# SuperbTUM/Faster-Distributed-Training

Measured on AMD Instinct MI355X. Metric: images/sec (whole node) ResNet-50 bs=1024 DDP at 1/2/4/8 MI355X; epoch time, higher is better.
Workload: dtype bf16; 1 GPU; model=resnet50 (CIFAR stem, 10 classes), global_batch=1024, image_size=32, parallelism=dp1, optimizer=madgrad, mixup=input, native_kernels=True, hip_graphs=True, deterministic=False

## Files before the change

### csrc/api.h

```cpp
#pragma once
#include <cstdint>
#include <vector>

namespace fdt {
void act_affine_fwd(uint64_t x, uint64_t s, uint64_t t, uint64_t out, long M, int C, int act, float alpha, int dt_in,
                    int dt_out, uint64_t stream);
int stats_num_blocks(long M, int C);
void set_ew_unroll(bool on);
void channel_stats_partial(uint64_t y, uint64_t part, long M, int C, int dt, uint64_t stream);
void stats_finalize(uint64_t part, int nb, int C, double count, int mode, float eps, float momentum, uint64_t gamma,
                    uint64_t beta, uint64_t run_mean, uint64_t run_var, uint64_t nbt, uint64_t out_s, uint64_t out_t,
                    uint64_t save_mean, uint64_t save_aux, int zero_after, uint64_t stream);
void bn_frozen_coef(uint64_t table, int units, uint64_t out, uint64_t stream);
void act_bwd_reduce(uint64_t g, uint64_t x, uint64_t s, uint64_t t, uint64_t gx, uint64_t part, int part_rows, long M,
                    int C, int act, float alpha, int dt, uint64_t stream);
void reduce_partials(uint64_t part, int nb, int nq, int C, uint64_t out, int zero_after, uint64_t stream);
int partials_compact(uint64_t part, int nb, int W, int R, uint64_t out, uint64_t stream);
void stats_bwd_coef(uint64_t gs, uint64_t gt, int C, double count, int mode, float eps, uint64_t save_mean,
                    uint64_t save_aux, uint64_t gamma, uint64_t alpha, uint64_t beta, uint64_t ggamma, uint64_t gbeta,
                    uint64_t stream);
void stats_bwd_finalize(uint64_t part, int nb, int nq, int C, int a_mode, float a_eps, double a_count, uint64_t a_sm,
                        uint64_t a_sa, uint64_t a_gamma, uint64_t a_alpha, uint64_t a_beta, uint64_t a_gg,
                        uint64_t a_gb, int b_mode, float b_eps, double b_count, uint64_t b_sm, uint64_t b_sa,
                        uint64_t b_gamma, uint64_t b_alpha, uint64_t b_beta, uint64_t b_gg, uint64_t b_gb,
// ... 83 lines not shown
void colsum_bf16(uint64_t x, uint64_t out, long rows, int cols, long ld, uint64_t stream);
void slab_sum_acc(uint64_t src, uint64_t dst, int s, long ld, long n, uint64_t stream);
void relu_bwd_colsum(uint64_t gact, uint64_t pre, uint64_t gpre, uint64_t gb, long rows, int cols, int dt,
                     uint64_t stream);
void augment(uint64_t src, uint64_t idx, uint64_t labels_src, uint64_t labels_out, uint64_t out, int B, int H, int W,
             int C, int Cout, int pad, int do_flip, uint64_t rng, float m0, float m1, float m2, float s0, float s1,
             float s2, int nchw, int pad_norm, int dt_out, uint64_t stream);
void rng_advance(uint64_t rng, uint64_t stream);
void conv_igemm(uint64_t x, uint64_t x2, uint64_t ps, uint64_t pt, uint64_t pg, uint64_t w, uint64_t out, uint64_t part,
                int part_rows, uint64_t ex, uint64_t es, uint64_t et, uint64_t jmask, uint64_t jyb, uint64_t jout, long Nb, int Hi,
                int Wi, int Cx, int Ho, int Wo, int S, const std::vector<int>& dh, const std::vector<int>& dw,
                const std::vector<int>& wt, int Cout, int ldw, int Hout, int Wout, int OS, int oy, int ox, int pro,
                int pro_act, float pro_alpha, int epi, int epi_act, float epi_alpha, int BM, int BN, int BK, int nsplit,
                uint64_t slab, uint64_t cnt, int kg, uint64_t stream, const std::vector<uint64_t>& jz);
void conv_igemm_join(uint64_t y, uint64_t r, uint64_t s, uint64_t t, uint64_t s2, uint64_t t2, uint64_t w, uint64_t out,
                     uint64_t part, int part_rows, uint64_t jout, uint64_t jmask, long Nb, int H, int W, int Cx, int Cout,
                     int ldw, int BM, int BN, int BK, int nsplit, uint64_t slab, uint64_t cnt, int kg, uint64_t stream);
void ffn_gemm(uint64_t x, uint64_t w, uint64_t out, long M, int K, int N, int epi, uint64_t bias, uint64_t out2,
              uint64_t a_in, uint64_t gb, float p, uint64_t seed, uint64_t seed_ptr, int BM, int BN, int BK, int kg,
              uint64_t stream);
int conv_num_row_blocks(long M, int BM);
void set_conv_write_through(bool on);
void set_conv_debug_flags(int f);
std::vector<long> conv_splitk_workspace(long M, int Cout, int BM, int BN, int nsplit);
void conv_wgrad(uint64_t g, uint64_t y, uint64_t al, uint64_t be, uint64_t gs, uint64_t x, uint64_t xs, uint64_t xt,
                uint64_t slab,
                long Nb, int Hi, int Wi, int Cx, int Ho, int Wo, int S, const std::vector<int>& dh,
                const std::vector<int>& dw, int Cout, int ldw, int act, float act_alpha, int BM, int BN, int BK,
                int nsplit, int direct, int stages, uint64_t out, uint64_t cnt, int Cin, int accumulate,
                uint64_t stream);
void wgrad_reduce(uint64_t slab, uint64_t out, int nsplit, int Cout, int Cin, int ntaps, int Cxp, int accumulate,
                  uint64_t stream);
void conv_bwd_pair(uint64_t g, uint64_t y, uint64_t al, uint64_t be, uint64_t gs, uint64_t wd, uint64_t x, uint64_t xs,
                   uint64_t xt, uint64_t es, uint64_t et, uint64_t dx, uint64_t part, int part_rows, uint64_t dw,
                   uint64_t slab, long M, int Cin, int Cout, int epi, int act, int wgs, int accumulate,
                   uint64_t stream);
bool conv_bwd_pair_supported(int Cin, int Cout, int epi, int act, int xaff);
void pack_weights(const std::vector<uint64_t>& src, const std::vector<uint64_t>& wf, const std::vector<uint64_t>& wd,
                  const std::vector<int>& cout, const std::vector<int>& cin, const std::vector<int>& cxp,
                  const std::vector<int>& ntaps, uint64_t stream);
void jacobi_eigh(uint64_t A, uint64_t w, uint64_t V, uint64_t table, int batch, int n, int max_sweeps, float tol, uint64_t stream);
void attn_fwd(uint64_t q, uint64_t k, uint64_t v, const std::vector<long>& strides, uint64_t out, uint64_t out32,
              uint64_t lse, uint64_t mask, int B, int L, int H, float fill, float p_drop, uint64_t seed,
              uint64_t seed_ptr, uint64_t stream);
void attn_bwd(uint64_t q, uint64_t k, uint64_t v, const std::vector<long>& strides, uint64_t o32, uint64_t dout,
              uint64_t lse, uint64_t delta, uint64_t mask, uint64_t dq, uint64_t dk, uint64_t dv, int B, int L, int H,
// ... 32 lines not shown
```

### csrc/bindings.cpp

```cpp
#include <pybind11/pybind11.h>
#include <pybind11/stl.h>

#include "api.h"
#include "runtime/runtime_api.h"

namespace py = pybind11;

namespace fdt {
const char* source_hash();
}

PYBIND11_MODULE(_fdt_native, m) {
  m.doc() = "MI355X (gfx950) HIP kernels and native runtime of faster_distributed_training_amd";
  m.attr("arch") = "gfx950";
  m.def("source_hash", &fdt::source_hash, "sha256 of the csrc/ sources this binary was built from");
#define DEF(name) m.def(#name, &fdt::name)
  DEF(act_affine_fwd);
  DEF(stats_num_blocks);
  DEF(set_ew_unroll);
  DEF(channel_stats_partial);
  DEF(stats_finalize);
  DEF(bn_frozen_coef);
  DEF(act_bwd_reduce);
  DEF(reduce_partials);
  DEF(partials_compact);
  DEF(stats_bwd_coef);
  DEF(stats_bwd_finalize);
  DEF(affine_fold);
  DEF(residual_act_fwd);
  DEF(residual_act_bwd);
  DEF(set_deterministic_mode);
  DEF(deterministic_mode);
  DEF(conv_igemm);
  DEF(conv_igemm_join);
  DEF(ffn_gemm);
  DEF(conv_num_row_blocks);
  DEF(set_conv_write_through);
  DEF(set_conv_debug_flags);
  DEF(conv_splitk_workspace);
  DEF(conv_wgrad);
  DEF(wgrad_reduce);
  DEF(conv_bwd_pair);
  DEF(conv_bwd_pair_supported);
  DEF(pack_weights);
  DEF(jacobi_eigh);
  DEF(ngd_pre_eigh);
  DEF(ngd_sumsq);
  DEF(ngd_small_supported);
  DEF(ngd_small_proj);
  DEF(ngd_small_part_numel);
  DEF(ngd_proj_supported);
  DEF(ngd_mfma);
  DEF(ngd_proj);
  DEF(ngd_proj_hbuf_numel);
  DEF(ngd_rescale);
  DEF(ngd_gram_slab_numel);
  DEF(ngd_gram);
  DEF(ngd_wupdate);
  DEF(ngd_post_eigh);
  DEF(attn_fwd);
  DEF(attn_bwd);
// ... 50 lines not shown
```

### csrc/kernels/conv_h3.hip

```cpp
#include "conv_igemm_impl.h"

namespace fdt {
namespace conv {

constexpr int kH3Taps = 9;
constexpr int kH3Row = 16;

__device__ __forceinline__ void h3_dma16(__amdgpu_buffer_rsrc_t r, void* lds, uint32_t off) {
  __builtin_amdgcn_raw_ptr_buffer_load_lds(r, (__attribute__((address_space(3))) void*)lds, 16, off, 0, 0, 0);
}

template <int BM>
constexpr int h3_halo_rows_max() {
  return BM / 16 * 36;
}

struct H3Geom {
  int W, Rb, W2, bhr, NI, GW, SPR;
  __device__ __forceinline__ H3Geom(int W_, int H_, int BM) {
    W = W_;
    Rb = H_ < BM / W_ ? H_ : BM / W_;
    W2 = W_ + 2;
    GW = W_ < 16 ? W_ : 16;
    NI = 16 / GW;
    SPR = W_ / GW;
    int b = (Rb + 2) * W2;
    if (NI > 1) b += ((16 / NI) - b % 16 + 16) % 16;
    bhr = b;
  }
  __device__ __forceinline__ int pix(int blk, int n) const {
    const int pn = n < 4 ? n : n < 12 ? n + 12 : n < 16 ? n - 8 : n < 20 ? n + 8 : n < 28 ? n - 12 : n;
    const int s = blk * 2 + (pn >> 4), i = pn & 15;
    const int per = Rb * SPR;
    const int gi = s / per, rr = s - gi * per, r = rr / SPR, seg = rr - r * SPR;
    const int img = NI * gi + i / GW, col = seg * GW + i % GW;
    return img * (Rb * W) + r * W + col;
  }
  static __device__ __forceinline__ int elem(int q, int h) { return q * kH3Row + 8 * (h ^ ((q >> 3) & 1)); }
  __device__ __forceinline__ int halo_row(int p) const {
    const int b = p / (Rb * W), r = (p / W) % Rb, c = p % W;
    return b * bhr + (r + 1) * W2 + c + 1;
  }
};

template <int BM, int BN, int WM, int WN, int TP = kH3Taps>
constexpr size_t h3_stage_elems() { return (size_t)TP * BN * 16 + (size_t)h3_halo_rows_max<BM>() * kH3Row; }

template <int BM, int BN, int EPI, int ACT, int WM, int WN, bool DMA, int NS = 2, int TP = kH3Taps>
__global__ __launch_bounds__(64 * WM * WN, (NS == 1 || BN == 64) ? 4 : 1) void h3_kernel(const ConvArgs a) {
  static_assert(NS == 2 || (NS == 1 && DMA), "single-stage: LDS-DMA staging");
  constexpr int NT = 64 * WM * WN;
  constexpr int TN = BN / WN / 32, TM = BM / WM / 32;
  static_assert(TN >= 1 && TM >= 1, "wave tile >= 32x32");
  constexpr int WP = TP * BN * 2;
  constexpr int NWP = (WP + NT - 1) / NT;
  constexpr int HRM = h3_halo_rows_max<BM>();
  constexpr int NHP = (2 * HRM + NT - 1) / NT;
  constexpr int NQ = EPI == kEpiJoinBwd ? 3 : 2;
  constexpr int WTILE = TP * BN * 16;
  constexpr int STAGE = (int)h3_stage_elems<BM, BN, WM, WN, TP>();

  extern __shared__ __attribute__((aligned(16))) char smem[];
  float* red = reinterpret_cast<float*>(smem);
  int* ttab = reinterpret_cast<int*>(red + (NT / 64) * NQ * BN);
  constexpr int HDR = (((NT / 64) * NQ * BN + 2 * kH3Taps) * 4 + 15) & ~15;
  bf16* tiles = reinterpret_cast<bf16*>(smem + HDR);
// ... 317 lines not shown
```

### csrc/kernels/conv_igemm.hip

```cpp
#include "conv_igemm_impl.h"

#include <algorithm>

namespace fdt {

static void conv_igemm_impl(uint64_t x, uint64_t x2, uint64_t ps, uint64_t pt, uint64_t pg, uint64_t w, uint64_t out,
                            uint64_t part, int part_rows, uint64_t ex, uint64_t es, uint64_t et, uint64_t jmask,
                            uint64_t jyb, uint64_t jout, long Nb, int Hi, int Wi, int Cx, int Ho, int Wo, int S,
                            const std::vector<int>& dh, const std::vector<int>& dw, const std::vector<int>& wt, int Cout,
                            int ldw, int Hout, int Wout, int OS, int oy, int ox, int pro, int pro_act, float pro_alpha,
                            int epi, int epi_act, float epi_alpha, int BM, int BN, int BK, int nsplit, uint64_t slab,
                            uint64_t cnt, uint64_t pt2, uint64_t pout, uint64_t pmask, int kg, uint64_t stream,
                            const std::vector<uint64_t>& jz = {}) {
  using namespace conv;
  ConvArgs a{};
  a.pt2 = P<const float>(pt2);
  a.pout = P<bf16>(pout);
  a.pmask = P<uint8_t>(pmask);
  if (pro == kProJoin) {
    FDT_CHECK(x2 != 0 && pout != 0 && ps != 0 && pt != 0 && (pg == 0 || pt2 != 0),
              "join prologue: y, r, s, t, out");
    FDT_CHECK(dh.size() == 1 && S == 1 && Hi == Ho && Wi == Wo, "join prologue: 1x1 stride-1 convolution only");
  }
  a.x = P<const bf16>(x);
// ... 55 lines not shown
  {
    const int nkt = (a.K + BK - 1) / BK;
    if (nsplit < 1 || nkt <= 1) nsplit = 1;
    if (nsplit > nkt && nkt >= 1) nsplit = nkt;
    a.kps = nsplit == 1 ? (nkt > 1 ? nkt : 1) : (nkt + nsplit - 1) / nsplit;
    a.nsplit = nsplit == 1 ? 1 : (nkt + a.kps - 1) / a.kps;
    a.slab = P<float>(slab);
    a.cnt = P<int>(cnt);
    FDT_CHECK(a.nsplit == 1 || (slab != 0 && cnt != 0), "split-K needs a slab and a zeroed ticket buffer");
  }
  const bool pure = a.ntaps == 1 && dh[0] == 0 && dw[0] == 0 && wt[0] == 0 && S == 1 && Hi == Ho && Wi == Wo;
  hipStream_t st = as_stream(stream);
  if (a.M == 0) return;
  if (epi == kEpiNormAct) {
    FDT_CHECK(pro == kProNone && es != 0 && et != 0, "frozen epilogue: prologue-free, with scale and shift");
    FDT_CHECK(OS == 1 && oy == 0 && ox == 0 && Hout == Ho && Wout == Wo, "frozen epilogue: dense forward output");
  }
  const int act = (pro == kProAffineAct || pro == kProJoin)
                      ? pro_act
                      : ((epi == kEpiActBwd || epi == kEpiJoinBwd || epi == kEpiNormAct) ? epi_act : 0);
  if (kg >= 5 && kg <= 8) {
    FDT_CHECK(pro == kProNone && a.nsplit == 1, "kg 5-8 (halo 3x3): prologue-free, nsplit 1");
    FDT_CHECK(launch_h3(pro, epi, act, a, BM, BN, kg, st), "kg 5-8 (halo 3x3): unsupported tile / epilogue");
    return;
  }
  if (kg == 10) {
    FDT_CHECK(launch_x1(pro, epi, act, a, BM, BN, xn, pure, st),
              "kg 10 (stationary 1x1): 1x1 stride-1, prologue none / affine (ReLU, none) / fold, epilogue "
              "STATS / STORE / ADD / ReLU-mask JOINBWD, tile 128x128 | 64x128, K a multiple of 64 within LDS, "
              "xn dividing Cout / BN");
    return;
  }
  if (kg == 2 && a.nsplit > 1) kg = 1;
  if (kg == 3 && pro != kProNone) kg = 1;
  if (launch_cases_fwd(pro, epi, act, a, BM, BN, BK, kg, pure, st) ||
      launch_cases_fold(pro, epi, act, a, BM, BN, BK, kg, pure, st) ||
      launch_cases_join(pro, epi, act, a, BM, BN, BK, kg, pure, st) ||
      launch_cases_plain(pro, epi, act, a, BM, BN, BK, kg, pure, st) ||
      launch_cases_infer(pro, epi, act, a, BM, BN, BK, kg, pure, st) ||
      launch_cases_ffn(pro, epi, act, a, BM, BN, BK, kg, pure, st))
    return;
  FDT_CHECK(false, "unsupported (prologue, epilogue) combination");
}

void conv_igemm(uint64_t x, uint64_t x2, uint64_t ps, uint64_t pt, uint64_t pg, uint64_t w, uint64_t out, uint64_t part,
                int part_rows, uint64_t ex, uint64_t es, uint64_t et, uint64_t jmask, uint64_t jyb, uint64_t jout, long Nb, int Hi,
// ... 78 lines not shown
```

### csrc/kernels/conv_igemm_impl.h

```cpp
#pragma once
#include "common.h"
#include "bn_math.h"
#include "dropout_math.h"
#include <vector>

namespace fdt {
namespace conv {

typedef short bf16x8_t __attribute__((ext_vector_type(8)));
typedef float f32x16 __attribute__((ext_vector_type(16)));

enum Pro : int { kProNone = 0, kProAffineAct = 1, kProFold = 2, kProJoin = 3 };
enum Epi : int { kEpiStats = 0, kEpiActBwd = 1, kEpiStore = 2, kEpiAdd = 3, kEpiJoinBwd = 4, kEpiGeluFwd = 5,
                 kEpiGeluBwd = 6, kEpiNormAct = 7 };

struct ConvArgs {
  const bf16* x;
  const bf16* x2;
  const float* ps;
  const float* pt;
  const float* pg;
  const float* pt2;
  bf16* pout;
  uint8_t* pmask;
// ... 103 lines not shown
  return make_float4(__uint_as_float(v[0]), __uint_as_float(v[1]), __uint_as_float(v[2]), __uint_as_float(v[3]));
}

constexpr uint32_t kOOB = 0xFFFFFFF0u;

__device__ __forceinline__ void st_out(__amdgpu_buffer_rsrc_t r, uint32_t byte_off, bf16* p, const float* v, int wt) {
  if (wt) {
    u32x4_t u = {pack_bf16x2(v[0], v[1]), pack_bf16x2(v[2], v[3]), pack_bf16x2(v[4], v[5]), pack_bf16x2(v[6], v[7])};
    __builtin_amdgcn_raw_buffer_store_b128(u, r, byte_off, 0, 16);
  } else {
    Vec8<bf16>::store(p, v);
  }
}

template <int BM, int BN, int BK, int PRO, bool PURE>
constexpr int kMinWavesPerEU =
    (BM == 128 && BN == 128 && BK == 32 && (PRO == kProNone || (PRO == kProAffineAct && PURE))) ? 4
    : (BM == 128 && BN == 128 && (BK == 32 || (PRO != 2 && PRO != 3))) ? 3 : 1;

struct PixLinear {
  int wstride;
  __device__ __forceinline__ int operator()(int wm, int j, int n) const { return wm * wstride + j * 32 + n; }
};
template <int BM, int BN, int EPI, int ACT, int NT, int WM, int WN, class PixF = PixLinear>
__device__ __forceinline__ void conv_epilogue(const ConvArgs& a, f32x16 (&acc)[BN / WN / 32][BM / WM / 32], long m0,
                                              int n0, int bm, int tid, float* stg, float* red, bool ew,
                                              float inv_alpha, PixF pix = PixLinear{BM / WM}) {
  constexpr int TN = BN / WN / 32, TM = BM / WM / 32;
  constexpr int NQ = EPI == kEpiJoinBwd ? 3 : 2;
  constexpr int SW = BN + 4;
  constexpr int CG = BN / 8;
  constexpr int RPS = NT / CG;
  constexpr int NSW = WM * 32 / RPS;
  static_assert(NSW >= 1 && NSW * RPS == WM * 32, "epilogue sweep geometry");
  constexpr int NW = NT / 64;
  const int lane = tid & 63, wid = tid >> 6, wn = wid % WN, wm = wid / WN;
  constexpr bool STATS = EPI == kEpiStats || EPI == kEpiActBwd || EPI == kEpiJoinBwd;
  const int h = lane >> 5;
  const __amdgpu_buffer_rsrc_t ro = __builtin_amdgcn_make_buffer_rsrc(
      (void*)a.out, (short)0, (int)0xFFFFFFFF, 0x00020000);
  const int cg = tid % CG, rs = tid / CG;
  const int c = n0 + cg * 8;
  const bool dense = a.OS == 1 && a.oy == 0 && a.ox == 0 && a.Hout == a.Ho && a.Wout == a.Wo;
  float sv[8], tv[8];
  constexpr bool GELU = EPI == kEpiGeluFwd || EPI == kEpiGeluBwd;
  uint64_t dseed = 0;
  if constexpr (GELU) dseed = drop::live_seed(a.drop_seed, a.drop_seed_ptr);
  if constexpr (EPI == kEpiGeluFwd) {
    const float4* bp = reinterpret_cast<const float4*>(a.fbias + c);
    const float4 b0 = bp[0], b1 = bp[1];
// ... 42 lines not shown
    for (int sw = 0; sw < NSW; ++sw) {
      const int lr = rs + sw * RPS;
      const long m = m0 + pix(lr >> 5, j, lr & 31);
      if (ew && m < a.M) {
        uint32_t orow;
        if (dense) {
          orow = (uint32_t)m;
        } else {
          const int mi = (int)m, hw = a.Ho * a.Wo;
          const int n = mi / hw, rem = mi - n * hw;
          const int oh = rem / a.Wo, ow = rem - oh * a.Wo;
          orow = (uint32_t)((n * a.Hout + oh * a.OS + a.oy) * a.Wout + ow * a.OS + a.ox);
        }
        const uint32_t e = orow * (uint32_t)a.Cout + c;
        const float4 va = *reinterpret_cast<const float4*>(stg + lr * SW + cg * 8);
        const float4 vb = *reinterpret_cast<const float4*>(stg + lr * SW + cg * 8 + 4);
        float v[8] = {va.x, va.y, va.z, va.w, vb.x, vb.y, vb.z, vb.w};
        if constexpr (EPI == kEpiStats) {
#pragma unroll
          for (int k = 0; k < 8; ++k) { q0[k] += v[k]; q1[k] = fmaf(v[k], v[k], q1[k]); }
          st_out(ro, e * 2u, a.out + e, v, a.wthru);
        } else if constexpr (EPI == kEpiActBwd) {
          float x8[8];
          Vec8<bf16>::load(a.ex + e, x8);
#pragma unroll
          for (int k = 0; k < 8; ++k) {
            const float gp = v[k] * actg<ACT>(fmaf(x8[k], sv[k], tv[k]), inv_alpha);
            v[k] = gp * sv[k];
            q0[k] = fmaf(gp, x8[k], q0[k]);
            q1[k] += gp;
          }
          st_out(ro, e * 2u, a.out + e, v, a.wthru);
        } else if constexpr (EPI == kEpiJoinBwd) {
          float e8[8], ya[8], yb[8], o8[8];
          Vec8<bf16>::load(a.out + e, e8);
          Vec8<bf16>::load(a.ex + e, ya);
          const bool hb = a.jyb != nullptr;
          if (hb) Vec8<bf16>::load(a.jyb + e, yb);
          uint32_t mk = 0;
          if constexpr (ACT == kActRelu) mk = a.jmask[e >> 3];
          else if (!zm) Vec8<bf16>::load(a.jout + e, o8);
          else if (!hb) Vec8<bf16>::load(a.jx + e, o8);
#pragma unroll
          for (int k = 0; k < 8; ++k) {
            const float gv = v[k] + e8[k];
            float gp;
            if constexpr (ACT == kActRelu) {
// ... 637 lines not shown
  if constexpr (PRO == kProJoin) {
    FDT_T(64, 256, 64) FDT_T(128, 256, 32) FDT_T(128, 256, 64)
  }
#undef FDT_T
#undef FDT_T2
  FDT_CHECK(false, "unsupported conv tile");
}


bool launch_cases_fwd(int pro, int epi, int act, const ConvArgs& a, int BM, int BN, int BK, int kg, bool pure,
                      hipStream_t st);
bool launch_cases_fold(int pro, int epi, int act, const ConvArgs& a, int BM, int BN, int BK, int kg, bool pure,
                       hipStream_t st);
bool launch_cases_join(int pro, int epi, int act, const ConvArgs& a, int BM, int BN, int BK, int kg, bool pure,
                       hipStream_t st);
bool launch_cases_plain(int pro, int epi, int act, const ConvArgs& a, int BM, int BN, int BK, int kg, bool pure,
                        hipStream_t st);
bool launch_cases_ffn(int pro, int epi, int act, const ConvArgs& a, int BM, int BN, int BK, int kg, bool pure,
                      hipStream_t st);
bool launch_cases_infer(int pro, int epi, int act, const ConvArgs& a, int BM, int BN, int BK, int kg, bool pure,
                        hipStream_t st);
bool h3_supported(const ConvArgs& a, int BM);
bool launch_h3(int pro, int epi, int act, const ConvArgs& a, int BM, int BN, int kg, hipStream_t st);
bool x1_supported(int pro, int epi, int act, const ConvArgs& a, int BM, int BN, int xn, bool pure);
bool launch_x1(int pro, int epi, int act, const ConvArgs& a, int BM, int BN, int xn, bool pure, hipStream_t st);

}
}
```

### faster_distributed_training_amd/ops/conv_igemm.py

```python
from __future__ import annotations

import json
import os
from dataclasses import dataclass
from functools import lru_cache

import torch

from . import _native

PRO_NONE, PRO_AFFINE_ACT, PRO_FOLD, PRO_JOIN = 0, 1, 2, 3
EPI_STATS, EPI_ACTBWD, EPI_STORE, EPI_ADD, EPI_JOINBWD = 0, 1, 2, 3, 4
EPI_NORMACT = 7


def _sp():
    return _native.stream_ptr()


def _p(t):
    return 0 if t is None else t.data_ptr()


def pad_channels(c: int) -> int:
# ... 114 lines not shown
        return tile[0], tile[1], 64
    return tuple(tile[:3])


WG_STAGES = int(os.environ.get("FDT_WG_STAGES", "2"))
WG_FUSED_REDUCE = os.environ.get("FDT_WG_FUSED_REDUCE", "0") == "1"
WG_FUSED_MAX_SPLITS = 8

KGROUPS = os.environ.get("FDT_KGROUPS", "1") != "0"
KG_TILES = {(128, 128, 64), (128, 64, 64), (64, 128, 64), (64, 64, 64), (64, 64, 128)}


GLDS = os.environ.get("FDT_CONV_GLDS", "0") == "1"


LOOP = os.environ.get("FDT_CONV_LOOP", "old")

H3 = os.environ.get("FDT_CONV_H3", "1") == "1"
H3_MIN_TILES = int(os.environ.get("FDT_CONV_H3_MIN_TILES", "256"))
H3_TILES = {(256, 128), (256, 64), (128, 128)}
H3_LOOP = os.environ.get("FDT_CONV_H3_LOOP", "auto")
H3_KGS = (5, 6, 7, 8)
H3_S2 = os.environ.get("FDT_CONV_H3_S2", "0") == "1"


def _h3_kg(kg, W=8):
    if kg in H3_KGS:
        return kg
    return {"dma": 6, "dma64": 6, "auto": 6, "dma1": 7}.get(H3_LOOP, 5)


def h3_tile(N, H, W, shp: "ConvShape", pro, cout, force=False, cx=None, bn=None, s2cls=False):
    if cx is None:
        cx = shp.cxp
    conv_ok = shp.k == 3 and shp.pad == 1 and shp.stride == (2 if s2cls else 1)
    if not (H3 or force) or pro != PRO_NONE or cx % 16 or not conv_ok or W < 4 or W & (W - 1):
        return None
    bm = 256
    M = N * H * W
    if M % bm or bm % W:
        return None
    rb = min(H, bm // W)
    if (rb < H and H % rb) or (rb == H and bm % (H * W)):
        return None
    nbk, gw = bm // (rb * W), min(W, 16)
    ni = 16 // gw
    bhr = (rb + 2) * (W + 2)
    if ni > 1:
        bhr += ((16 // ni) - bhr % 16 + 16) % 16
        if nbk % ni or rb != H:
            return None
    elif W % 16:
        return None
    if nbk * bhr > bm // 16 * 36:
        return None
    if bn is None:
        bn = 64 if H3_LOOP == "dma64" else 128
    bn = bn if cout % bn == 0 else (64 if cout % 64 == 0 else 0)
    if not bn or (not force and (M // bm) * (cout // bn) < H3_MIN_TILES):
        return None
    return bm, bn


def h3_auto(N, H, W, shp: "ConvShape", pro, cout, cx=None):
    if H3_LOOP != "auto":
        t = h3_tile(N, H, W, shp, pro, cout, cx=cx)
        return None if t is None else (t, _h3_kg(None, W))
    if h3_tile(N, H, W, shp, pro, cout, force=True, cx=cx, bn=64) is None:
        return None
    tiles128 = (N * H * W // 256) * (cout // 128) if cout % 128 == 0 else 0
    if W >= 32:
        return (256, 64), 6
    if W >= 8:
        if tiles128 >= 512:
            return (256, 128), 7
        return ((256, 64), 6) if W >= 16 else None
    return ((256, 128), 6) if tiles128 >= 256 else None


def _loop_kg(ent, kgv):
    lp = (ent.get("loop") if ent else None) or LOOP
    return 4 if (kgv == 1 and lp == "rot") else kgv


X1_KG = 10
X1_BN = 128
X1_BM_OF_K = {64: 128, 128: 128, 256: 128, 512: 64}
X1_LDS_MAX = 80 * 1024


def x1_lds_bytes(pro, epi, K, bn=X1_BN):
    nprm = {PRO_FOLD: 3, PRO_AFFINE_ACT: 2}.get(pro, 0)
    nq = 3 if epi == EPI_JOINBWD else 2
    hdr = ((nprm * K + 4 * nq * bn) * 4 + 15) & ~15
# ... 83 lines not shown

def conv_fwd(x, wf, shp: ConvShape, s=None, t=None, act=0, alpha=1.0, tile=None, part=None, nsplit=None,
             fin=None, kg=None, norm=None, res=None, out_act=None, xn=None, out=None):
    nat = _native.native()
    N, H, W, C = x.shape
    assert C == shp.cxp and x.dtype == torch.bfloat16 and x.is_contiguous()
    Ho, Wo = out_hw(H, W, shp)
    M = N * Ho * Wo
    frozen = norm is not None
    if frozen:
        assert s is None and t is None and act == 0 and part is None and fin is None, \
            "frozen epilogue: prologue-free, no statistics"
        es, et = norm
        for v in (es, et):
            assert v.dtype == torch.float32 and v.is_contiguous() and v.numel() == shp.cout and v.device == x.device
        assert res is None or (res.dtype == torch.bfloat16 and res.is_contiguous() and res.device == x.device
                               and tuple(res.shape) == (N, Ho, Wo, shp.cout))
        oact, oalpha = out_act if out_act is not None else (0, 1.0)
    else:
        assert res is None and out_act is None, "res / out_act belong to the frozen epilogue (norm=)"
    pro = PRO_AFFINE_ACT if (s is not None or act != 0) else PRO_NONE
    ent = None
    h3 = None
    if kg in H3_KGS:
        t3 = h3_tile(N, H, W, shp, pro, shp.cout, True)
        h3 = None if t3 is None else (t3, kg)
    elif kg is None and tile is None and H3:
        h3 = h3_auto(N, H, W, shp, pro, shp.cout)
    if tile is None and h3 is None:
        ent = tuned(f"fwd{pro}", N, H, shp) or tuned("fwd", N, H, shp)
        tile = tuple(ent["tile"]) if ent else None
    if h3 is not None:
        ent, ((bm, bn), kgv), bk = {"loop": "old"}, h3, 16
        ns, slab_p, cnt_p = 1, 0, 0
    else:
        bm, bn, bk = _tile3(tile, M, shp.cout)
        if nsplit is not None:
            ent = dict(ent or {}, nsplit=nsplit) if frozen else {"nsplit": nsplit}
        ns, slab_p, cnt_p = _splitk_args(ent, M, shp.cout, shp.ntaps * C, bm, bn, bk, x.device)
        xn = int(xn if xn is not None else (ent or {}).get("xn", 1))
        x1 = x1_ok(_is_pure(shp), pro, EPI_NORMACT if frozen else EPI_STATS, int(act), shp.ntaps * C, shp.cout,
                   bm, bn, xn)
        kgv = _kg(ent, kg, (bm, bn, bk), ns, shp.ntaps * C, pro, x1)
    _log("fwd", N, H, shp, ent, (bm, bn, bk), ns, kgv)
    if kgv == X1_KG:
        ns, slab_p, cnt_p = xn, 0, 0
    if out is None:
        y = torch.empty(N, Ho, Wo, shp.cout, device=x.device, dtype=torch.bfloat16)
    else:
        y = out
        assert y.dtype == torch.bfloat16 and y.is_contiguous() and tuple(y.shape) == (N, Ho, Wo, shp.cout)
    dh, dw, wt = taps_fwd(shp.k, shp.pad)
    if frozen:
        nat.conv_igemm(x.data_ptr(), 0, 0, 0, 0, wf.data_ptr(), y.data_ptr(), 0, 0,
                       _p(res), es.data_ptr(), et.data_ptr(), 0, 0, 0,
                       N, H, W, C, Ho, Wo, shp.stride, list(dh), list(dw), list(wt), shp.cout, shp.ntaps * shp.cxp,
                       Ho, Wo, 1, 0, 0, PRO_NONE, 0, 1.0, EPI_NORMACT, int(oact), float(oalpha), bm, bn, bk, ns, slab_p,
                       cnt_p, _loop_kg(ent, kgv), _sp(), [])
        return y, None
    if part is None:
        part = stat_slots(2, shp.cout, x.device, M)
    if pro == PRO_AFFINE_ACT and s is None:
        s = torch.ones(C, device=x.device, dtype=torch.float32)
        t = torch.zeros(C, device=x.device, dtype=torch.float32)
    nat.conv_igemm(x.data_ptr(), 0, _p(s), _p(t), 0, wf.data_ptr(), y.data_ptr(), part.data_ptr(), part.shape[0],
                   0, 0, 0, 0, 0, 0,
                   N, H, W, C, Ho, Wo, shp.stride, list(dh), list(dw), list(wt), shp.cout, shp.ntaps * shp.cxp,
                   Ho, Wo, 1, 0, 0, pro, int(act), float(alpha), EPI_STATS, 0, 1.0, bm, bn, bk, ns, slab_p, cnt_p,
                   _loop_kg(ent, kgv), _sp(), [])
# ... 35 lines not shown

def conv_dgrad(g, y, al, be, wd, shp: ConvShape, x_shape, epi=EPI_STORE, out=None, ex=None, es=None, et=None,
               act=0, alpha=1.0, tile=None, part=None, nsplit=None, gs=None, jmask=None, jyb=None, jout=None,
               coef=None, kg=None, jz=None, xn=None):
    nat = _native.native()
    N, Hy, Wy, Cy = g.shape
    assert Cy == shp.cout and g.is_contiguous() and (y is None or y.is_contiguous())
    Nx, Hx, Wx, Cx = x_shape
    assert Cx == shp.cin
    if out is None:
        out = torch.empty(N, Hx, Wx, shp.cin, device=g.device, dtype=torch.bfloat16)
    if epi == EPI_ACTBWD and part is None:
        part = stat_slots(2, shp.cin, g.device, Nx * Hx * Wx)
    if epi == EPI_JOINBWD:
        assert shp.stride == 1 and ex is not None and part is not None and (
            jmask is not None or jout is not None or jz is not None)
        assert (jz is None) == (es is None), "z mode: es / et with jz"
        if jz is not None:
            assert act == 2 and et is not None and len(jz) == 3
            assert (jz[0] is not None and jz[1] is not None) if jyb is not None else jz[2] is not None
            if jz[2] is not None:
                assert jz[2].dtype == torch.bfloat16 and jz[2].is_contiguous() and tuple(jz[2].shape) == tuple(x_shape)
    ent = None
    h3ok = kg in H3_KGS or (kg is None and tile is None)
    if tile is None:
        pro = PRO_FOLD if al is not None else PRO_NONE
        e = EPI_STORE if epi in (EPI_ADD, EPI_JOINBWD) else epi
        ent = ((tuned(f"dgrad{pro}{epi}", N, Hx, shp) if e != epi else None)
               or tuned(f"dgrad{pro}{e}", N, Hx, shp) or tuned("dgrad", N, Hx, shp))
        tile = tuple(ent["tile"]) if ent else None
    if nsplit is not None:
        ent = {"nsplit": nsplit}
    classes = dgrad_classes(shp.k, shp.stride, shp.pad)
    assert coef is None or epi in (EPI_ACTBWD, EPI_JOINBWD)
    for (py, px, dh, dw, wt) in classes:
        Ha = (Hx - py + shp.stride - 1) // shp.stride
        Wa = (Wx - px + shp.stride - 1) // shp.stride
        M = N * Ha * Wa
        if len(dh) == 0 and epi == EPI_ADD:
            continue
        pro = PRO_FOLD if al is not None else PRO_NONE
        h3 = None
        if h3ok and epi in (EPI_ACTBWD, EPI_STORE) and len(dh) == 9:
            if kg in H3_KGS:
                t3 = h3_tile(N, Hx, Wx, shp, pro, shp.cin, True, cx=Cy)
                h3 = None if t3 is None else (t3, kg)
            elif H3:
                h3 = h3_auto(N, Hx, Wx, shp, pro, shp.cin, cx=Cy)
        elif (h3ok and epi in (EPI_ACTBWD, EPI_STORE) and len(dh) in (2, 4) and shp.k == 3 and shp.stride == 2
              and Ha == Hy and Wa == Wy and (H3_S2 or kg in H3_KGS)):
            t3 = h3_tile(N, Ha, Wa, shp, pro, shp.cin, force=kg in H3_KGS, cx=Cy, s2cls=True)
            h3 = None if t3 is None else (t3, 6)
        if h3 is not None:
            ((bm, bn), kgv), bk = h3, 16
            ns, slab_p, cnt_p = 1, 0, 0
        else:
            bm, bn, bk = _tile3(tile, M, shp.cin)
            ns, slab_p, cnt_p = _splitk_args(ent, M, shp.cin, len(dh) * Cy, bm, bn, bk, g.device)
            xnv = int(xn if xn is not None else (ent or {}).get("xn", 1))
            x1 = x1_ok(_is_pure(shp), pro, epi, int(act) if epi == EPI_JOINBWD else 0, len(dh) * Cy, shp.cin,
                       bm, bn, xnv, relu_mask=jmask is not None and jz is None)
            kgv = _kg(ent, kg, (bm, bn, bk), ns, len(dh) * Cy, pro, x1)
        _log("dgrad", N, Hx, shp, ent, (bm, bn, bk), ns, kgv)
        if kgv == X1_KG:
            ns, slab_p, cnt_p = xnv, 0, 0
        assert gs is None or pro == PRO_FOLD, "gs needs the fold prologue (al/be)"
        nat.conv_igemm(g.data_ptr(), _p(y) if pro == PRO_FOLD else 0, _p(al), _p(be), _p(gs), wd.data_ptr(),
                       out.data_ptr(), _p(part) if epi in (EPI_ACTBWD, EPI_JOINBWD) else 0,
                       part.shape[0] if part is not None else 0, _p(ex), _p(es), _p(et),
                       _p(jmask), _p(jyb), _p(jout), N, Hy, Wy, Cy, Ha, Wa, 1,
                       list(dh), list(dw), list(wt), shp.cin, shp.ntaps * shp.cout, Hx, Wx, shp.stride, py, px,
                       pro, 0, 1.0, epi, int(act), float(alpha), bm, bn, bk, ns, slab_p, cnt_p, _loop_kg(ent, kgv),
                       _sp(), [_p(v) for v in jz] if jz is not None else [])
    if coef is not None:
        _finalize_standalone(nat, 2, part, 3 if epi == EPI_JOINBWD else 2, shp.cin, coef[0], coef[1])
    return out, (part if epi in (EPI_ACTBWD, EPI_JOINBWD) else None)


WH3 = os.environ.get("FDT_WGRAD_H3", "1") == "1"
WH3_WGS = int(os.environ.get("FDT_WGRAD_H3_WGS", "256"))
WH3_MIN_CPS = int(os.environ.get("FDT_WGRAD_H3_MIN_CPS", "1"))
WH3_PX = 128
WH3_PIPE = os.environ.get("FDT_WGRAD_H3_PIPE", "0") == "1"
WH3_TS = int(os.environ.get("FDT_WGRAD_H3_TS", "1"))


def wh3_plan(N, H, W, shp: "ConvShape", cx, fold=False, xaff=False, force=False):
    if not (WH3 or force) or fold or xaff or shp.k != 3 or shp.stride != 1 or shp.pad != 1:
# ... 178 lines not shown
```

Before: 44150 images/sec.

## Add persistent halo 3x3 conv kernel with resident weights and double-buffered halo

Adds a persistent-grid 3x3 stride-1 conv kernel for 64->64 channel, 32-wide layers. Each CU-sized workgroup loads the full weight set into LDS once, then loops over tiles while DMA-prefetching the next tile's halo into a second buffer. For ACTBWD it also prefetches the epilogue activation input into registers. The kernel is selected automatically in h3_auto when there are enough tiles. This removes repeated weight loads and per-tile launch and prologue latency, at the cost of a large LDS footprint (one workgroup per CU) and fixed-shape restrictions.

```diff
diff --git a/csrc/api.h b/csrc/api.h
--- a/csrc/api.h
+++ b/csrc/api.h
@@ -129,6 +129,7 @@
 int conv_num_row_blocks(long M, int BM);
 void set_conv_write_through(bool on);
 void set_conv_debug_flags(int f);
+void set_conv_h3p_wgs(int wgs);
 std::vector<long> conv_splitk_workspace(long M, int Cout, int BM, int BN, int nsplit);
 void conv_wgrad(uint64_t g, uint64_t y, uint64_t al, uint64_t be, uint64_t gs, uint64_t x, uint64_t xs, uint64_t xt,
                 uint64_t slab,
diff --git a/csrc/bindings.cpp b/csrc/bindings.cpp
--- a/csrc/bindings.cpp
+++ b/csrc/bindings.cpp
@@ -37,6 +37,7 @@
   DEF(conv_num_row_blocks);
   DEF(set_conv_write_through);
   DEF(set_conv_debug_flags);
+  DEF(set_conv_h3p_wgs);
   DEF(conv_splitk_workspace);
   DEF(conv_wgrad);
   DEF(wgrad_reduce);
diff --git a/csrc/kernels/conv_h3.hip b/csrc/kernels/conv_h3.hip
--- a/csrc/kernels/conv_h3.hip
+++ b/csrc/kernels/conv_h3.hip
@@ -1,47 +1,12 @@
-#include "conv_igemm_impl.h"
+#include "conv_h3_geom.h"
 
 namespace fdt {
 namespace conv {
-
-constexpr int kH3Taps = 9;
-constexpr int kH3Row = 16;
-
-__device__ __forceinline__ void h3_dma16(__amdgpu_buffer_rsrc_t r, void* lds, uint32_t off) {
-  __builtin_amdgcn_raw_ptr_buffer_load_lds(r, (__attribute__((address_space(3))) void*)lds, 16, off, 0, 0, 0);
-}
 
 template <int BM>
 constexpr int h3_halo_rows_max() {
   return BM / 16 * 36;
 }
-
-struct H3Geom {
-  int W, Rb, W2, bhr, NI, GW, SPR;
-  __device__ __forceinline__ H3Geom(int W_, int H_, int BM) {
-    W = W_;
-    Rb = H_ < BM / W_ ? H_ : BM / W_;
-    W2 = W_ + 2;
-    GW = W_ < 16 ? W_ : 16;
-    NI = 16 / GW;
-    SPR = W_ / GW;
-    int b = (Rb + 2) * W2;
-    if (NI > 1) b += ((16 / NI) - b % 16 + 16) % 16;
-    bhr = b;
-  }
-  __device__ __forceinline__ int pix(int blk, int n) const {
-    const int pn = n < 4 ? n : n < 12 ? n + 12 : n < 16 ? n - 8 : n < 20 ? n + 8 : n < 28 ? n - 12 : n;
-    const int s = blk * 2 + (pn >> 4), i = pn & 15;
-    const int per = Rb * SPR;
-    const int gi = s / per, rr = s - gi * per, r = rr / SPR, seg = rr - r * SPR;
-    const int img = NI * gi + i / GW, col = seg * GW + i % GW;
-    return img * (Rb * W) + r * W + col;
-  }
-  static __device__ __forceinline__ int elem(int q, int h) { return q * kH3Row + 8 * (h ^ ((q >> 3) & 1)); }
-  __device__ __forceinline__ int halo_row(int p) const {
-    const int b = p / (Rb * W), r = (p / W) % Rb, c = p % W;
-    return b * bhr + (r + 1) * W2 + c + 1;
-  }
-};
 
 template <int BM, int BN, int WM, int WN, int TP = kH3Taps>
 constexpr size_t h3_stage_elems() { return (size_t)TP * BN * 16 + (size_t)h3_halo_rows_max<BM>() * kH3Row; }
diff --git a/csrc/kernels/conv_h3_geom.h b/csrc/kernels/conv_h3_geom.h
--- /dev/null
+++ b/csrc/kernels/conv_h3_geom.h
@@ -0,0 +1,43 @@
+#pragma once
+#include "conv_igemm_impl.h"
+
+namespace fdt {
+namespace conv {
+
+constexpr int kH3Taps = 9;
+constexpr int kH3Row = 16;
+
+__device__ __forceinline__ void h3_dma16(__amdgpu_buffer_rsrc_t r, void* lds, uint32_t off) {
+  __builtin_amdgcn_raw_ptr_buffer_load_lds(r, (__attribute__((address_space(3))) void*)lds, 16, off, 0, 0, 0);
+}
+
+struct H3Geom {
+  int W, Rb, W2, bhr, NI, GW, SPR;
+  __device__ __forceinline__ H3Geom(int W_, int H_, int BM) {
+    W = W_;
+    Rb = H_ < BM / W_ ? H_ : BM / W_;
+    W2 = W_ + 2;
+    GW = W_ < 16 ? W_ : 16;
+    NI = 16 / GW;
+    SPR = W_ / GW;
+    int b = (Rb + 2) * W2;
+    if (NI > 1) b += ((16 / NI) - b % 16 + 16) % 16;
+    bhr = b;
+  }
+  __device__ __forceinline__ int pix(int blk, int n) const {
+    const int pn = n < 4 ? n : n < 12 ? n + 12 : n < 16 ? n - 8 : n < 20 ? n + 8 : n < 28 ? n - 12 : n;
+    const int s = blk * 2 + (pn >> 4), i = pn & 15;
+    const int per = Rb * SPR;
+    const int gi = s / per, rr = s - gi * per, r = rr / SPR, seg = rr - r * SPR;
+    const int img = NI * gi + i / GW, col = seg * GW + i % GW;
+    return img * (Rb * W) + r * W + col;
+  }
+  static __device__ __forceinline__ int elem(int q, int h) { return q * kH3Row + 8 * (h ^ ((q >> 3) & 1)); }
+  __device__ __forceinline__ int halo_row(int p) const {
+    const int b = p / (Rb * W), r = (p / W) % Rb, c = p % W;
+    return b * bhr + (r + 1) * W2 + c + 1;
+  }
+};
+
+}
+}
diff --git a/csrc/kernels/conv_h3p.hip b/csrc/kernels/conv_h3p.hip
--- /dev/null
+++ b/csrc/kernels/conv_h3p.hip
@@ -0,0 +1,246 @@
+#include "conv_h3_geom.h"
+
+namespace fdt {
+namespace conv {
+
+namespace {
+constexpr int kPBM = 256, kPBN = 64, kPWM = 4, kPWN = 2, kPNT = 64 * kPWM * kPWN, kPTM = kPBM / kPWM / 32;
+constexpr int kPW = 32, kPRb = kPBM / kPW, kPW2 = kPW + 2, kPHR = (kPRb + 2) * kPW2;
+constexpr int kPC = 64, kPCh = kPC / 16;
+constexpr int kPHdr = 80;
+constexpr int kPWPlane = kH3Taps * kPBN * 16 * 2;
+constexpr int kPWBytes = kPCh * kPWPlane;
+constexpr int kPHPlane = kPHR * kH3Row * 2;
+constexpr int kPHPieces = kPCh * kPHR * 2;
+constexpr int kPHInstr = (kPHPieces + 63) / 64;
+constexpr int kPHBuf = kPHInstr * 1024;
+constexpr int kPStage = kPWM * 32 * (kPBN + 4) * 4;
+constexpr int kPRed = (kPNT / 64) * 2 * kPBN * 4;
+constexpr int kPLds = kPHdr + kPWBytes + 2 * kPHBuf;
+static_assert(kPStage + kPRed <= kPHBuf, "epilogue staging + statistics alias one halo buffer");
+static_assert(kPLds <= 160 * 1024, "LDS budget");
+static_assert(kPWPlane % 1024 == 0, "whole 1-KiB weight DMA pieces");
+
+struct PixH3P {
+  H3Geom g;
+  __device__ __forceinline__ int operator()(int wm_, int j, int n) const { return g.pix(wm_ + kPWM * j, n); }
+};
+
+int& h3p_wgs_ref() {
+  static int v = 0;
+  return v;
+}
+}
+
+template <int EPI, int ACT>
+__global__ __launch_bounds__(kPNT, 1) void h3p_kernel(const ConvArgs a) {
+  constexpr int NW = kPNT / 64;
+  const int ntiles = a.nbm;
+  if ((int)blockIdx.x >= ntiles) return;
+
+  extern __shared__ __attribute__((aligned(16))) char smem[];
+  int* ttab = reinterpret_cast<int*>(smem);
+  char* wts = smem + kPHdr;
+  char* ring = wts + kPWBytes;
+
+  const int tid = threadIdx.x, lane = tid & 63, wid = tid >> 6;
+  const int wn = wid % kPWN, wm = wid / kPWN;
+  const int wv = __builtin_amdgcn_readfirstlane(wid);
+  const float inv_alpha = ACT == kActCelu ? 1.f / a.epi_alpha : 1.f;
+  const H3Geom geo(kPW, a.Hi, kPBM);
+
+  if (tid < kH3Taps) {
+    ttab[tid] = a.wt[tid];
+    ttab[kH3Taps + tid] = a.dh[tid] * kPW2 + a.dw[tid];
+  }
+  __syncthreads();
+
+  const __amdgpu_buffer_rsrc_t rx_d = __builtin_amdgcn_make_buffer_rsrc((void*)a.x, (short)0,
+                                                                        (int)(a.Nb_HiWi_Cx_bytes), 0x00020000);
+  const __amdgpu_buffer_rsrc_t rw_d = __builtin_amdgcn_make_buffer_rsrc((void*)a.w, (short)0, (int)(a.w_bytes),
+                                                                        0x00020000);
+
+  {
+    constexpr int IPP = kPWPlane / 1024;
+#pragma unroll
+    for (int j = 0; j < kPCh * IPP / NW; ++j) {
+      const int wi = j * NW + wv;
+      const int ch = wi / IPP, piece = (wi - ch * IPP) * 64 + lane;
+      const int tap = piece / (2 * kPBN), rem = piece - tap * 2 * kPBN;
+      const int n = rem >> 1, lh = (rem & 1) ^ ((n >> 3) & 1);
+      const uint32_t src = ((uint32_t)n * (uint32_t)a.ldw + (uint32_t)(ttab[tap] * kPC + 16 * ch + 8 * lh)) * 2u;
+      h3_dma16(rw_d, wts + wi * 1024, src);
+    }
+  }
+  static_assert(kPCh * (kPWPlane / 1024) % NW == 0, "weight pieces divide over the waves");
+
+  constexpr int NHJ = (kPHInstr + NW - 1) / NW;
+  int hpk[NHJ];
+#pragma unroll
+  for (int j = 0; j < NHJ; ++j) {
+    const int piece = (j * NW + wv) * 64 + lane;
+    const int ch = piece / (2 * kPHR), rem = piece - ch * 2 * kPHR;
+    const int q = rem >> 1, part = (rem & 1) ^ ((q >> 3) & 1);
+    const int hr = q / kPW2, hc = q - hr * kPW2;
+    const bool v = piece < kPHPieces && hc >= 1 && hc <= kPW;
+    const int cls = !v ? 0 : hr == 0 ? 2 : hr == kPRb + 1 ? 3 : 1;
+    hpk[j] = (((hr - 1) * kPW + hc - 1) * (kPC * 2) + ch * 32 + part * 16) | cls;
+  }
+  const int hmask = (a.Hi >> 3) - 1;
+  auto issue = [&](int tile, int buf) {
+    const uint32_t base = (uint32_t)tile * (uint32_t)(kPBM * kPC * 2);
+    const int tr = tile & hmask;
+    const bool top = tr == 0, bot = tr == hmask;
+    char* dst = ring + buf * kPHBuf;
+#pragma unroll
+    for (int j = 0; j < NHJ; ++j) {
+      const int wi = j * NW + wv;
+      if (wi < kPHInstr) {
+        const int cls = hpk[j] & 3;
+        const bool ok = cls == 1 || (cls == 2 && !top) || (cls == 3 && !bot);
+        h3_dma16(rx_d, dst + wi * 1024, ok ? base + (uint32_t)(hpk[j] & ~15) : kOOB);
+      }
+    }
+  };
+
+  const int h = lane >> 5;
+  int xoff[kH3Taps][kPTM];
+#pragma unroll
+  for (int j = 0; j < kPTM; ++j) {
+    const int qb = geo.halo_row(geo.pix(wm + kPWM * j, lane & 31));
+#pragma unroll
+    for (int t = 0; t < kH3Taps; ++t) xoff[t][j] = H3Geom::elem(qb + ttab[kH3Taps + t], h) * 2;
+  }
+  const int arow = wn * 32 + (lane & 31);
+  const int aoff = (arow * 16 + 8 * (h ^ ((lane >> 3) & 1))) * 2;
+
+  constexpr bool PRE = EPI == kEpiActBwd;
+  constexpr int NEX = PRE ? 2 * kPTM : 1;
+  int exoff[NEX];
+  if constexpr (PRE) {
+    const PixH3P px{geo};
+#pragma unroll
+    for (int j = 0; j < kPTM; ++j)
+#pragma unroll
+      for (int sw = 0; sw < 2; ++sw) {
+        const int lr = tid / (kPBN / 8) + sw * (kPNT / (kPBN / 8));
+        exoff[j * 2 + sw] = px(lr >> 5, j, lr & 31) * kPBN + (tid % (kPBN / 8)) * 8;
+      }
+  }
+  static_assert(kPWM * 32 / (kPNT / (kPBN / 8)) == 2, "two sweeps per epilogue pass");
+
+  const bool no_dma = a.dbg & 2, no_mma = a.dbg & 4, no_epi = a.dbg & 8;
+  const int grid = gridDim.x;
+  issue(xcd_remap(blockIdx.x, ntiles), 0);
+  asm volatile("s_waitcnt vmcnt(0)" ::: "memory");
+  __syncthreads();
+  for (int k = 0;; ++k) {
+    const int vb = blockIdx.x + k * grid;
+    const int tile = xcd_remap(vb, ntiles);
+    const int buf = k & 1;
+    const bool more = vb + grid < ntiles;
+    if (more && !no_dma) issue(xcd_remap(vb + grid, ntiles), buf ^ 1);
+    ExRegs<NEX> exq;
+    if constexpr (PRE) {
+      const bf16* exb = a.ex + (long)tile * (kPBM * kPBN);
+#pragma unroll
+      for (int i = 0; i < NEX; ++i) exq.u[i] = *reinterpret_cast<const uint4*>(exb + exoff[i]);
+    }
+
+    f32x16 acc[1][kPTM];
+#pragma unroll
+    for (int j = 0; j < kPTM; ++j)
+#pragma unroll
+      for (int r = 0; r < 16; ++r) acc[0][j][r] = 0.f;
+
+    const char* Hl = ring + buf * kPHBuf;
+    bf16x8_t wf[2], xf[2][kPTM];
+    auto fetch = [&](int s, int sl) {
+      const int c = s / kH3Taps, t = s - c * kH3Taps;
+      wf[sl] = *reinterpret_cast<const bf16x8_t*>(wts + c * kPWPlane + t * (kPBN * 32) + aoff);
+#pragma unroll
+      for (int j = 0; j < kPTM; ++j)
+        xf[sl][j] = *reinterpret_cast<const bf16x8_t*>(Hl + c * kPHPlane + xoff[t][j]);
+    };
+    if (!no_mma) {
+    fetch(0, 0);
+#pragma unroll
+    for (int s = 0; s < kPCh * kH3Taps; ++s) {
+      const int sl = s & 1;
+      if (s + 1 < kPCh * kH3Taps) fetch(s + 1, sl ^ 1);
+      __builtin_amdgcn_sched_barrier(0);
+#pragma unroll
+      for (int j = 0; j < kPTM; ++j)
+        acc[0][j] = __builtin_amdgcn_mfma_f32_32x32x16_bf16(wf[sl], xf[sl][j], acc[0][j], 0, 0, 0);
+      __builtin_amdgcn_sched_barrier(0);
+    }
+    }
+
+    asm volatile("s_waitcnt vmcnt(0)" ::: "memory");
+    char* stg = ring + buf * kPHBuf;
+    if (no_epi) __syncthreads();
+    else if constexpr (PRE)
+      conv_epilogue<kPBM, kPBN, EPI, ACT, kPNT, kPWM, kPWN, PixH3P, ExRegs<NEX>>(
+          a, acc, (long)tile * kPBM, 0, tile, tid, reinterpret_cast<float*>(stg),
+          reinterpret_cast<float*>(stg + kPStage), true, inv_alpha, PixH3P{geo}, exq);
+    else
+      conv_epilogue<kPBM, kPBN, EPI, ACT, kPNT, kPWM, kPWN, PixH3P>(
+          a, acc, (long)tile * kPBM, 0, tile, tid, reinterpret_cast<float*>(stg),
+          reinterpret_cast<float*>(stg + kPStage), true, inv_alpha, PixH3P{geo});
+    if (!more) break;
+    asm volatile("s_waitcnt lgkmcnt(0)" ::: "memory");
+    __builtin_amdgcn_s_barrier();
+    asm volatile("" ::: "memory");
+  }
+}
+
+template <int EPI, int ACT>
+static void h3p_launch_one(const ConvArgs& a, int grid, hipStream_t st) {
+  auto kern = h3p_kernel<EPI, ACT>;
+  static bool attr = false;
+  if (!attr) {
+    FDT_HIP_CHECK(hipFuncSetAttribute(reinterpret_cast<const void*>(kern), hipFuncAttributeMaxDynamicSharedMemorySize,
+                                      kPLds));
+    attr = true;
+  }
+  hipLaunchKernelGGL(kern, dim3(grid), dim3(kPNT), kPLds, st, a);
+  FDT_LAUNCH_CHECK();
+}
+
+bool h3p_supported(int pro, int epi, int act, const ConvArgs& a, int BM, int BN) {
+  if (pro != kProNone || BM != kPBM || BN != kPBN || a.ntaps != kH3Taps || !h3_supported(a, BM)) return false;
+  if (a.Cx != kPC || a.Cout != kPBN || a.Wi != kPW || a.Hi < kPRb || (a.Hi & (a.Hi - 1)) != 0) return false;
+  return ((epi == kEpiStats || epi == kEpiStore) && act == kActNone) ||
+         (epi == kEpiActBwd && (act == kActRelu || act == kActCelu)) ||
+         (epi == kEpiNormAct && (act == kActNone || act == kActRelu || act == kActCelu));
+}
+
+bool launch_h3p(int pro, int epi, int act, const ConvArgs& a, int BM, int BN, hipStream_t st) {
+  if (!h3p_supported(pro, epi, act, a, BM, BN)) return false;
+  static int cus = 0;
+  if (cus == 0) {
+    int dev = 0;
+    FDT_HIP_CHECK(hipGetDevice(&dev));
+    FDT_HIP_CHECK(hipDeviceGetAttribute(&cus, hipDeviceAttributeMultiprocessorCount, dev));
+    FDT_CHECK(cus > 0, "persistent halo 3x3 conv: CU count");
+  }
+  const int want = h3p_wgs_ref() > 0 ? h3p_wgs_ref() : cus;
+  const int grid = want < a.nbm || h3p_wgs_ref() > 0 ? want : a.nbm;
+#define FDT_H3P(E_, A_) \
+  if (epi == E_ && act == A_) { h3p_launch_one<E_, A_>(a, grid, st); return true; }
+  FDT_H3P(kEpiStats, kActNone)
+  FDT_H3P(kEpiActBwd, kActRelu)
+  FDT_H3P(kEpiActBwd, kActCelu)
+  FDT_H3P(kEpiStore, kActNone)
+  FDT_H3P(kEpiNormAct, kActNone)
+  FDT_H3P(kEpiNormAct, kActRelu)
+  FDT_H3P(kEpiNormAct, kActCelu)
+#undef FDT_H3P
+  return false;
+}
+
+}
+
+void set_conv_h3p_wgs(int wgs) { conv::h3p_wgs_ref() = wgs > 0 ? wgs : 0; }
+
+}
diff --git a/csrc/kernels/conv_igemm.hip b/csrc/kernels/conv_igemm.hip
--- a/csrc/kernels/conv_igemm.hip
+++ b/csrc/kernels/conv_igemm.hip
@@ -101,6 +101,12 @@
   if (kg >= 5 && kg <= 8) {
     FDT_CHECK(pro == kProNone && a.nsplit == 1, "kg 5-8 (halo 3x3): prologue-free, nsplit 1");
     FDT_CHECK(launch_h3(pro, epi, act, a, BM, BN, kg, st), "kg 5-8 (halo 3x3): unsupported tile / epilogue");
+    return;
+  }
+  if (kg == 11) {
+    FDT_CHECK(a.nsplit == 1 && launch_h3p(pro, epi, act, a, BM, BN, st),
+              "kg 11 (persistent halo 3x3): dense 3x3 stride-1, 64 -> 64 channels, 32-wide images of a power-of-two "
+              "height >= 8, tile 256x64, prologue-free, epilogue STATS / STORE / ACTBWD / NORMACT");
     return;
   }
   if (kg == 10) {
diff --git a/csrc/kernels/conv_igemm_impl.h b/csrc/kernels/conv_igemm_impl.h
--- a/csrc/kernels/conv_igemm_impl.h
+++ b/csrc/kernels/conv_igemm_impl.h
@@ -149,10 +149,23 @@
   int wstride;
   __device__ __forceinline__ int operator()(int wm, int j, int n) const { return wm * wstride + j * 32 + n; }
 };
-template <int BM, int BN, int EPI, int ACT, int NT, int WM, int WN, class PixF = PixLinear>
+struct ExLoad {
+  static constexpr bool kPre = false;
+  __device__ __forceinline__ void get(int, float*) const {}
+};
+template <int NR>
+struct ExRegs {
+  static constexpr bool kPre = true;
+  uint4 u[NR];
+  __device__ __forceinline__ void get(int i, float* v) const {
+    v[0] = bf16_lo(u[i].x); v[1] = bf16_hi(u[i].x); v[2] = bf16_lo(u[i].y); v[3] = bf16_hi(u[i].y);
+    v[4] = bf16_lo(u[i].z); v[5] = bf16_hi(u[i].z); v[6] = bf16_lo(u[i].w); v[7] = bf16_hi(u[i].w);
+  }
+};
+template <int BM, int BN, int EPI, int ACT, int NT, int WM, int WN, class PixF = PixLinear, class ExQ = ExLoad>
 __device__ __forceinline__ void conv_epilogue(const ConvArgs& a, f32x16 (&acc)[BN / WN / 32][BM / WM / 32], long m0,
                                               int n0, int bm, int tid, float* stg, float* red, bool ew,
-                                              float inv_alpha, PixF pix = PixLinear{BM / WM}) {
+                                              float inv_alpha, PixF pix = PixLinear{BM / WM}, const ExQ& exq = ExQ{}) {
   constexpr int TN = BN / WN / 32, TM = BM / WM / 32;
   constexpr int NQ = EPI == kEpiJoinBwd ? 3 : 2;
   constexpr int SW = BN + 4;
@@ -241,7 +254,8 @@
           st_out(ro, e * 2u, a.out + e, v, a.wthru);
         } else if constexpr (EPI == kEpiActBwd) {
           float x8[8];
-          Vec8<bf16>::load(a.ex + e, x8);
+          if constexpr (ExQ::kPre) exq.get(j * NSW + sw, x8);
+          else Vec8<bf16>::load(a.ex + e, x8);
 #pragma unroll
           for (int k = 0; k < 8; ++k) {
             const float gp = v[k] * actg<ACT>(fmaf(x8[k], sv[k], tv[k]), inv_alpha);
@@ -925,6 +939,8 @@
                         hipStream_t st);
 bool h3_supported(const ConvArgs& a, int BM);
 bool launch_h3(int pro, int epi, int act, const ConvArgs& a, int BM, int BN, int kg, hipStream_t st);
+bool h3p_supported(int pro, int epi, int act, const ConvArgs& a, int BM, int BN);
+bool launch_h3p(int pro, int epi, int act, const ConvArgs& a, int BM, int BN, hipStream_t st);
 bool x1_supported(int pro, int epi, int act, const ConvArgs& a, int BM, int BN, int xn, bool pure);
 bool launch_x1(int pro, int epi, int act, const ConvArgs& a, int BM, int BN, int xn, bool pure, hipStream_t st);
 
diff --git a/faster_distributed_training_amd/ops/conv_igemm.py b/faster_distributed_training_amd/ops/conv_igemm.py
--- a/faster_distributed_training_amd/ops/conv_igemm.py
+++ b/faster_distributed_training_amd/ops/conv_igemm.py
@@ -160,6 +160,11 @@
 H3_LOOP = os.environ.get("FDT_CONV_H3_LOOP", "auto")
 H3_KGS = (5, 6, 7, 8)
 H3_S2 = os.environ.get("FDT_CONV_H3_S2", "0") == "1"
+H3P = os.environ.get("FDT_CONV_H3P", "1")
+H3P_MIN_TILES = int(os.environ.get("FDT_CONV_H3P_MIN_TILES", "512"))
+H3P_WGS = int(os.environ.get("FDT_CONV_H3P_WGS", "0"))
+H3P_KG = 11
+H3P_TILE = (256, 64)
 
 
 def _h3_kg(kg, W=8):
@@ -200,6 +205,19 @@
     return bm, bn
 
 
+def h3p_ok(N, H, W, shp: "ConvShape", pro, cout, cx=None, epi=None, act=0):
+    if cx is None:
+        cx = shp.cxp
+    if cx != 64 or cout != 64 or W != 32 or H < 8 or H & (H - 1):
+        return False
+    if h3_tile(N, H, W, shp, pro, cout, force=True, cx=cx, bn=64) != H3P_TILE:
+        return False
+    if epi is None:
+        return True
+    return ((epi in (EPI_STATS, EPI_STORE) and act == 0) or (epi == EPI_ACTBWD and act in (1, 2))
+            or (epi == EPI_NORMACT and act in (0, 1, 2)))
+
+
 def h3_auto(N, H, W, shp: "ConvShape", pro, cout, cx=None):
     if H3_LOOP != "auto":
         t = h3_tile(N, H, W, shp, pro, cout, cx=cx)
@@ -208,6 +226,9 @@
         return None
     tiles128 = (N * H * W // 256) * (cout // 128) if cout % 128 == 0 else 0
     if W >= 32:
+        if (H3P == "force" or (H3P == "1" and N * H * W // 256 >= H3P_MIN_TILES)) and h3p_ok(
+                N, H, W, shp, pro, cout, cx=cx):
+            return H3P_TILE, H3P_KG
         return (256, 64), 6
     if W >= 8:
         if tiles128 >= 512:
@@ -337,7 +358,10 @@
     pro = PRO_AFFINE_ACT if (s is not None or act != 0) else PRO_NONE
     ent = None
     h3 = None
-    if kg in H3_KGS:
+    if kg == H3P_KG:
+        assert h3p_ok(N, H, W, shp, pro, shp.cout), "kg 11 (persistent halo 3x3): unsupported launch"
+        h3 = (H3P_TILE, kg)
+    elif kg in H3_KGS:
         t3 = h3_tile(N, H, W, shp, pro, shp.cout, True)
         h3 = None if t3 is None else (t3, kg)
     elif kg is None and tile is None and H3:
@@ -360,6 +384,8 @@
     _log("fwd", N, H, shp, ent, (bm, bn, bk), ns, kgv)
     if kgv == X1_KG:
         ns, slab_p, cnt_p = xn, 0, 0
+    if kgv == H3P_KG:
+        nat.set_conv_h3p_wgs(H3P_WGS)
     if out is None:
         y = torch.empty(N, Ho, Wo, shp.cout, device=x.device, dtype=torch.bfloat16)
     else:
@@ -441,7 +467,7 @@
             if jz[2] is not None:
                 assert jz[2].dtype == torch.bfloat16 and jz[2].is_contiguous() and tuple(jz[2].shape) == tuple(x_shape)
     ent = None
-    h3ok = kg in H3_KGS or (kg is None and tile is None)
+    h3ok = kg in H3_KGS or kg == H3P_KG or (kg is None and tile is None)
     if tile is None:
         pro = PRO_FOLD if al is not None else PRO_NONE
         e = EPI_STORE if epi in (EPI_ADD, EPI_JOINBWD) else epi
@@ -461,7 +487,11 @@
         pro = PRO_FOLD if al is not None else PRO_NONE
         h3 = None
         if h3ok and epi in (EPI_ACTBWD, EPI_STORE) and len(dh) == 9:
-            if kg in H3_KGS:
+            if kg == H3P_KG:
+                assert h3p_ok(N, Hx, Wx, shp, pro, shp.cin, cx=Cy, epi=epi, act=int(act)), \
+                    "kg 11 (persistent halo 3x3): unsupported launch"
+                h3 = (H3P_TILE, kg)
+            elif kg in H3_KGS:
                 t3 = h3_tile(N, Hx, Wx, shp, pro, shp.cin, True, cx=Cy)
                 h3 = None if t3 is None else (t3, kg)
             elif H3:
@@ -483,6 +513,8 @@
         _log("dgrad", N, Hx, shp, ent, (bm, bn, bk), ns, kgv)
         if kgv == X1_KG:
             ns, slab_p, cnt_p = xnv, 0, 0
+        if kgv == H3P_KG:
+            nat.set_conv_h3p_wgs(H3P_WGS)
         assert gs is None or pro == PRO_FOLD, "gs needs the fold prologue (al/be)"
         nat.conv_igemm(g.data_ptr(), _p(y) if pro == PRO_FOLD else 0, _p(al), _p(be), _p(gs), wd.data_ptr(),
                        out.data_ptr(), _p(part) if epi in (EPI_ACTBWD, EPI_JOINBWD) else 0,
```

New measurement: 44150 images/sec, median of 2. About the same (-0.0%).
